# visinf/veto

Hardware: AMD Instinct MI355X
Metric: relation-pairs/sec (PredCls, 36 obj/img) (higher is better)
Workload: dtype fp16 + e4m3 correction terms (fp16 MFMA main product, e4m3 K=128 MFMA cross terms, fp32 accumulate); 1 GPU; BASELINE.json configs[1]: synthetic PredCls, 12 img x 36 obj = 15120 pairs/GPU, d=576, 8 heads, 4 layers, 51 predicates; images_per_gpu=12, objects_per_image=36, pairs_per_gpu=15120, layers=4, heads=8, precision=mixed, parallelism=single GPU

## Files before the change

veto_amd/csrc/attention.hip:

```cpp
#include "common.h"
#include "kernels.h"

#include <cstdio>
#include <cstdlib>
#include <cstring>

namespace veto {

namespace {

constexpr int kWavesPerBlock = 4;

__global__ __launch_bounds__(256) void attention_kernel(AttnArgs a, int dh, int ldh ) {
  extern __shared__ __attribute__((aligned(16))) char smem_raw[];
  const int lane = threadIdx.x & 63, w = threadIdx.x >> 6;
  const long gw = (long)blockIdx.x * kWavesPerBlock + w;
  const int per_wave = 3 * kTokens * ldh + kTokens * 20;
  float* sq = (float*)smem_raw + (size_t)w * per_wave;
  float* sk = sq + kTokens * ldh;
  float* sv = sk + kTokens * ldh;
  float* sp = sv + kTokens * ldh;
  const bool active = gw < (long)a.n_pair * a.heads;
  const int pair = active ? (int)(gw / a.heads) : 0;
  const int head = active ? (int)(gw % a.heads) : 0;
// ... 72 lines not shown
typedef _Float16 att_f16x8 __attribute__((ext_vector_type(8)));
__device__ __forceinline__ f32x16 att_mfma(const u32x4& a, const u32x4& b, const f32x16& c) {
  return __builtin_amdgcn_mfma_f32_32x32x16_f16(__builtin_bit_cast(att_f16x8, a), __builtin_bit_cast(att_f16x8, b), c, 0, 0, 0);
}
typedef short att_s16x4 __attribute__((ext_vector_type(4)));
typedef short att_s16x8 __attribute__((ext_vector_type(8)));

template <int V> struct IntTag { static constexpr int value = V; };
template <int I, int N, class F>
__device__ __forceinline__ void att_static_for(F&& f) {
  if constexpr (I < N) {
    f(IntTag<I>());
    att_static_for<I + 1, N>(f);
  }
}
constexpr int kAttWpb = 2;
#ifdef VETO_ATT_STAMPS
__device__ unsigned long long g_att_stamps[8192 * 10];
#define ATT_T(k) do { __builtin_amdgcn_sched_barrier(0); unsigned long long t_; asm volatile("s_memtime %0\n\ts_waitcnt lgkmcnt(0)" : "=s"(t_)::"memory"); \
                      __builtin_amdgcn_sched_barrier(0); att_dt[k] = t_ - att_t; att_t = t_; } while (0)
#else
#define ATT_T(k)
#endif
template <int DH, bool TAB = false, bool F24 = false>
__global__ __launch_bounds__(64 * kAttWpb, TAB && DH > 72 ? 2 : 3) void attention_mfma_kernel(AttnArgs a) {
  static_assert(!(TAB && F24), "the per-object form reads fp32 tables");
  saturating_conversions_on();
#ifdef VETO_ATT_STAMPS
  unsigned long long att_t, att_dt[10] = {0, 0, 0, 0, 0, 0, 0, 0, 0, 0};
  asm volatile("s_memtime %0\n\ts_waitcnt lgkmcnt(0)" : "=s"(att_t)::"memory");
#endif
  constexpr int KS = (DH + 15) / 16;
  constexpr int RB = DH * 2 + (DH % 32 == 0 ? 16 : 0);
  constexpr int NT = (DH + 31) / 32;
  constexpr int QK_PLANE = kTokens * RB;
  constexpr int V_PLANE = (kTokens + 1) * RB;
  constexpr int O_BYTES = kTokens * DH * 4;
  constexpr int PHASE2 = 2 * V_PLANE + O_BYTES;
  constexpr int kConstBytes = TAB ? (3 * DH * 4 + 32 * 4) : 0;
  constexpr int kImgBytes = ((4 * QK_PLANE > PHASE2 ? 4 * QK_PLANE : PHASE2) + 64 + 15) & ~15;
  constexpr int WAVE_LDS = kImgBytes + kConstBytes;
  constexpr int CH = DH / 8;
  constexpr int PER_MAT = kTokens * CH;
  constexpr int ROUNDS = (3 * PER_MAT + 63) / 64;
  static_assert(DH % 8 == 0 && QK_PLANE % 16 == 0 && V_PLANE % 16 == 0, "layout");
  __shared__ __attribute__((aligned(16))) char smem[kAttWpb * WAVE_LDS];

  const int lane = threadIdx.x & 63, w = __builtin_amdgcn_readfirstlane(threadIdx.x >> 6);
  const long item = (long)blockIdx.x * kAttWpb + w;
  if (item >= (long)a.n_pair * a.heads) return;
  char* base = smem + w * WAVE_LDS;
  char* q_hi = base;
  char* q_lo = base + QK_PLANE;
  char* k_hi = base + 2 * QK_PLANE;
  char* k_lo = base + 3 * QK_PLANE;
  char* v_hi = base;
  char* v_lo = v_hi + V_PLANE;

  constexpr int PC = DH / 4;
  constexpr int PER_MAT4 = kTokens * PC;
  constexpr int ROUNDS4 = (3 * PER_MAT4 + 63) / 64;
  f32x4 ld[TAB ? 1 : ROUNDS][2];
  f32x4 lt[TAB ? ROUNDS4 : 1], lo_[TAB ? ROUNDS4 : 1];
  const int pair = (int)(item / a.heads);
  const int head = (int)(item % a.heads);
  const float* src0 = a.qkv + (size_t)pair * kTokens * (3 * kDim) + head * DH;
  const float* tab_s = nullptr;
  const float* tab_o = nullptr;
  if constexpr (TAB) {
    tab_s = a.sw + (size_t)a.subj[pair] * kPatchTokens * (3 * kDim) + head * DH;
    tab_o = a.ow + (size_t)a.obj[pair] * kPatchTokens * (3 * kDim) + head * DH;
  }
  constexpr int kLateFrom = TAB ? (2 * PER_MAT4 + 63) / 64 : ROUNDS;
  constexpr int kRounds = TAB ? ROUNDS4 : ROUNDS;
  float* const c2_lds = (float*)(base + kImgBytes);
  float* const rs_lds = c2_lds + 3 * DH;
  if constexpr (TAB) {
    constexpr int NC2 = 3 * DH / 4;
#pragma unroll
    for (int idx0 = 0; idx0 < NC2; idx0 += 64) {
      const int idx = idx0 + lane;
      if (idx < NC2) {
        const int mat = idx / PC, c4 = idx % PC;
        *(f32x4*)(c2_lds + idx * 4) = *(const f32x4*)(a.vec + head * DH + mat * kDim + c4 * 4);
      }
    }
    if (lane < kTokens) rs_lds[lane] = a.stats[((size_t)pair * kTokens + lane) * 2 + 1];
  }
  auto load_round = [&](auto r_tag) {
    constexpr int r = decltype(r_tag)::value;
    const int e = lane + 64 * r;
    if constexpr (TAB) {
      const int mat = e / PER_MAT4, rem = e % PER_MAT4, i = rem / PC, c4 = rem % PC;
      const bool need = e < 3 * PER_MAT4;
      lo_[r] = f32x4{0.f, 0.f, 0.f, 0.f};
      if (need && i >= 1 && i <= kPatchTokens) {
        const unsigned off = (unsigned)(((i - 1) * (3 * kDim) + mat * kDim + c4 * 4) * 4);
        lo_[r] = *(const f32x4*)((const char*)tab_o + off);
        lt[r] = *(const f32x4*)((const char*)tab_s + off);
      } else if (need) {
        const unsigned off = (unsigned)((mat * kDim + c4 * 4) * 4) + (i == 0 ? 0u : (unsigned)(i * (3 * kDim) * 4));
        const char* src = i == 0 ? (const char*)(a.vec + 2 * (3 * kDim) + head * DH) : (const char*)src0;
        lt[r] = *(const f32x4*)(src + off);
      } else {
        lt[r] = f32x4{0.f, 0.f, 0.f, 0.f};
      }
    } else {
    const int mat = e / PER_MAT, rem = e % PER_MAT, i = rem / CH, c = rem % CH;
    const bool need = e < 3 * PER_MAT && !(a.cls_only && mat == 0 && i > 0);
    if (F24 && need) {
      const char* src = (const char*)a.qkv + (((size_t)pair * kTokens + i) * (3 * kDim) + mat * kDim + head * DH + c * 8) * 3;
      typedef u32x4 u32x4_a8 __attribute__((aligned(8)));
      const u32x4 d01 = *(const u32x4_a8*)src;
      const u32x2 d2 = *(const u32x2*)(src + 16);
      ld[r][0] = f32x4{__uint_as_float(d01[0]), __uint_as_float(d01[1]), __uint_as_float(d01[2]), __uint_as_float(d01[3])};
      ld[r][1] = f32x4{__uint_as_float(d2[0]), __uint_as_float(d2[1]), 0.f, 0.f};
    } else if (need) {
      const unsigned off = (unsigned)((mat * kDim + c * 8) * 4) + (unsigned)(i * (3 * kDim) * 4);
      ld[r][0] = *(const f32x4*)((const char*)src0 + off);
      ld[r][1] = *(const f32x4*)((const char*)src0 + off + 16u);
    } else {
      ld[r][0] = f32x4{0.f, 0.f, 0.f, 0.f};
      ld[r][1] = f32x4{0.f, 0.f, 0.f, 0.f};
    }
    }
  };
  att_static_for<0, kLateFrom>(load_round);
  ATT_T(0);
  auto convert = [&](auto phase_tag) {
    constexpr int PHASE = decltype(phase_tag)::value;
    if constexpr (TAB) {
      att_static_for<0, ROUNDS4>([&](auto r_tag) {
        constexpr int r = decltype(r_tag)::value;
        if constexpr (!(PHASE == 0 ? r >= kLateFrom : 64 * r + 63 < 2 * PER_MAT4)) {
          const int e = lane + 64 * r;
          const int mat = e / PER_MAT4, rem = e % PER_MAT4, i = rem / PC, c4 = rem % PC;
          if (e < 3 * PER_MAT4) {
            if ((PHASE == 0 ? r < kLateFrom : r >= kLateFrom) && i >= 1 && i <= kPatchTokens)
              lt[r] = rs_lds[i] * (lt[r] + lo_[r]) + *(const f32x4*)(c2_lds + mat * DH + c4 * 4);
            if (PHASE == 0 ? mat < 2 : mat == 2) {
              uint32_t h0, l0, h1, l1;
              att_split2(lt[r][0], lt[r][1], h0, l0);
              att_split2(lt[r][2], lt[r][3], h1, l1);
              char* dst = (PHASE == 0 ? (mat == 0 ? q_hi : k_hi) : v_hi) + i * RB + c4 * 8;
              *(u32x2*)dst = u32x2{h0, h1};
              *(u32x2*)(dst + (PHASE == 0 ? QK_PLANE : V_PLANE)) = u32x2{l0, l1};
            }
          }
        }
      });
    } else {
#pragma unroll
    for (int r = 0; r < ROUNDS; ++r) {
      if (PHASE == 0 ? 64 * r >= 2 * PER_MAT : 64 * r + 63 < 2 * PER_MAT) continue;
      const int e = lane + 64 * r;
      if (e >= 3 * PER_MAT) continue;
      const int mat = e / PER_MAT, rem = e % PER_MAT, i = rem / CH, c = rem % CH;
      if (PHASE == 0 ? mat == 2 : mat < 2) continue;
      f32x4 v0 = ld[r][0], v1 = ld[r][1];
      if constexpr (F24) {
        v0 = unpack_f24x4(__float_as_uint(ld[r][0][0]), __float_as_uint(ld[r][0][1]), __float_as_uint(ld[r][0][2]));
        v1 = unpack_f24x4(__float_as_uint(ld[r][0][3]), __float_as_uint(ld[r][1][0]), __float_as_uint(ld[r][1][1]));
// ... 133 lines not shown
    const int i = e / CH, c = e % CH;
    const f32x4 v0 = *(const f32x4*)(o_lds + i * DH + c * 8);
    const f32x4 v1 = *(const f32x4*)(o_lds + i * DH + c * 8 + 4);
    const size_t row = a.cls_only ? (size_t)pair : (size_t)pair * kTokens + i;
    if (a.o_fmt == FMT_MIXED) {
      store_act8_mixed<true>(a.o + row * (2 * kDim), head * DH + c * 8, v0, v1);
      continue;
    }
    bf16x8 hi, lo;
#pragma unroll
    for (int t = 0; t < 4; ++t) {
      __bf16 hh, ll;
      split_bf16(v0[t], hh, ll);
      hi[t] = hh;
      lo[t] = ll;
      split_bf16(v1[t], hh, ll);
      hi[4 + t] = hh;
      lo[4 + t] = ll;
    }
    __bf16* dst = a.o + row * (2 * kDim) + split_index(head * DH + c * 8);
    *(bf16x8*)dst = hi;
    *(bf16x8*)(dst + 32) = lo;
  }
#ifdef VETO_ATT_STAMPS
  ATT_T(9);
  if (lane == 0) {
    unsigned long long* slot = g_att_stamps + (size_t)(item & 8191) * 10;
    for (int k = 0; k < 10; ++k) slot[k] = att_dt[k];
  }
#endif
}


template <int CTRL>
__device__ __forceinline__ float dpp_rot16(float v) {
  return __int_as_float(__builtin_amdgcn_update_dpp(0, __float_as_int(v), CTRL, 0xF, 0xF, false));
}
__device__ __forceinline__ float row16_sum(float v) {
  v += dpp_rot16<0x128>(v);
  v += dpp_rot16<0x124>(v);
  v += dpp_rot16<0x122>(v);
  v += dpp_rot16<0x121>(v);
  return v;
}

constexpr int kFoldMaxHeads = 12;
// ... 371 lines not shown
      fprintf(stderr, "[cls stamps]");
      for (int k = 1; k <= 12; ++k) fprintf(stderr, " %lld", (long long)(hst[k] - hst[k - 1]));
      fprintf(stderr, "  (request | zero | loads->LN start.. | LN+images | barrier | scores | barrier | softmax | barrier | abar | barrier | staging | stores)\n");
    }
  }
#endif
  return hipGetLastError();
}

bool attention_reads_tables(int heads) {
  if (heads <= 0 || kDim % heads != 0) return false;
  const int dh = kDim / heads;
  return dh == 72 || dh == 96;
}

hipError_t launch_attention(const AttnArgs& a, hipStream_t s) {
  if (kDim % a.heads != 0) return hipErrorInvalidValue;
  const int dh = kDim / a.heads;
  if (dh == 72 || dh == 96) {
    const long items = (long)a.n_pair * a.heads;
    unsigned blocks = (unsigned)((items + kAttWpb - 1) / kAttWpb);
    if (a.sw) {
      if (!a.ow || !a.stats || !a.vec || !a.subj || !a.obj || a.cls_only) return hipErrorInvalidValue;
      if (dh == 72) VETO_LAUNCH((attention_mfma_kernel<72, true>), dim3(blocks), dim3(64 * kAttWpb), 0, s, a);
      else VETO_LAUNCH((attention_mfma_kernel<96, true>), dim3(blocks), dim3(64 * kAttWpb), 0, s, a);
#ifdef VETO_ATT_STAMPS
      {
        static unsigned long long all[8192 * 10];
        unsigned long long host[10] = {0};
        hipDeviceSynchronize();
        hipMemcpyFromSymbol(all, HIP_SYMBOL(g_att_stamps), sizeof(all));
        const long nslots = items < 8192 ? items : 8192;
        for (long i = 0; i < nslots; ++i)
          for (int k = 0; k < 10; ++k) host[k] += all[i * 10 + k];
        const double n = (double)nslots;
        static const char* names[10] = {"issue of the early gathers", "wait for the early gathers", "table arithmetic + Q / K conversion", "issue of the late gathers",
                                        "S^T", "softmax", "wait for the late gathers", "V arithmetic + conversion", "P V + staging", "output conversion + stores"};
        double tot = 0;
        for (int k = 0; k < 10; ++k) tot += host[k] / n;
        fprintf(stderr, "[attention stamps, table form, dh %d, last %.0f items] mean shader-clock cycles per item (s_memtime) and share:\n", dh, n);
        for (int k = 0; k < 10; ++k) fprintf(stderr, "    %-38s %8.1f  %5.1f %%\n", names[k], host[k] / n, 100.0 * host[k] / n / tot);
        fprintf(stderr, "    %-38s %8.1f\n", "sum", tot);
      }
#endif
    } else if (a.qkv_f24) {
      if (dh == 72) VETO_LAUNCH((attention_mfma_kernel<72, false, true>), dim3(blocks), dim3(64 * kAttWpb), 0, s, a);
// ... 25 lines not shown
```

veto_amd/csrc/gemm_split_ps.hip:

```cpp
#include "common.h"
#include "kernels.h"

#include <cstdio>
#include <cstdlib>

namespace veto {

namespace {

constexpr int BM = 256, BN = 192, BK = 32;
constexpr int NCONS = 8, NLOAD = 4;
constexpr int kABytes = BM * 128;
constexpr int kWBytes = BN * 128;
constexpr int kDumpOff = 3 * kABytes + 2 * kWBytes;
constexpr int kBiasOff = kDumpOff + 1024;
constexpr int kBiasSlices = 3;
constexpr int kLdsBytes = kBiasOff + kBiasSlices * BN * 4;
constexpr int kPrefSteps = BN * 4 / 128;
constexpr int CPA = BM / 8 / NLOAD;
constexpr int CPWL = BN / 8 / NLOAD;
#ifndef VETO_GEMM_EPI_T
#define VETO_GEMM_EPI_T 1
#endif
constexpr bool kEpiT = VETO_GEMM_EPI_T;
// ... 21 lines not shown

__device__ __forceinline__ void wg_barrier() {
  asm volatile("" ::: "memory");
  __builtin_amdgcn_s_barrier();
  asm volatile("" ::: "memory");
}

typedef int i32x4 __attribute__((ext_vector_type(4)));
typedef int i32x8 __attribute__((ext_vector_type(8)));
typedef _Float16 f16x8 __attribute__((ext_vector_type(8)));
template <int V> struct IntTag { static constexpr int value = V; };

typedef short s16x4 __attribute__((ext_vector_type(4)));
typedef short s16x8 __attribute__((ext_vector_type(8)));
__device__ __forceinline__ s16x4 lds_tr16(const char* p) {
  return __builtin_amdgcn_ds_read_tr16_b64_v4i16((__attribute__((address_space(3))) s16x4*)p);
}
__device__ __forceinline__ bf16x8 lds_tr_frag(const char* p, int pitch4) {
  const s16x4 a = lds_tr16(p), b = lds_tr16(p + pitch4);
  const s16x8 v = __builtin_shufflevector(a, b, 0, 1, 2, 3, 4, 5, 6, 7);
  return __builtin_bit_cast(bf16x8, v);
}

template <int NTERMS, int EPI_T, bool TN = false>
__global__ __launch_bounds__(64 * (NCONS + NLOAD), 3) void gemm_split_ps_kernel(GemmArgs g) {
  constexpr bool kDrop = EPI_T == EPI_RESID_DROP;
  constexpr bool kMixed = NTERMS == 2;
  if constexpr (kMixed) saturating_conversions_on();
  static_assert(!(kMixed && TN), "the mixed-row format has no transposed (weight-gradient) form");
  constexpr bool kGeluBwd = EPI_T == EPI_GELU_BWD;
  constexpr int EPI = kDrop || kGeluBwd ? (int)EPI_RESID : EPI_T;
  __shared__ __attribute__((aligned(16))) char smem[kLdsBytes];

  const int tid = threadIdx.x;
  const int lane = tid & 63;
  const int w = __builtin_amdgcn_readfirstlane(tid >> 6);
  const int b = blockIdx.x;
  const int ksp = EPI == EPI_ATOMIC && g.k_splits > 1 ? g.k_splits : 1;
  const int out_tiles = g.tiles_m * g.tiles_n;
  const int ntiles = out_tiles * ksp;
  const int K = g.K;
  const int nk = g.kb_tiles > 0 ? g.kb_steps : K / BK / ksp;
  const int per_xcd = gridDim.x >> 3;
  auto tile_of = [&](int it) { return (it * 8 + (b & 7)) * per_xcd + (b >> 3); };
  int my_tiles = 0;
  while (tile_of(my_tiles) < ntiles) ++my_tiles;
  if (my_tiles == 0) return;
// ... 18 lines not shown
      tn_xa[0] = (lane ^ tn_swz(lw)) << 4;
      tn_xa[1] = (lane ^ tn_swz(lw + 8)) << 4;
#pragma unroll
      for (int i = 0; i < CPWL; ++i) {
        const int slot = (lw + NLOAD * i) * 64 + lane, r = slot / 48, cc = slot % 48;
        tn_wr[i] = r;
        tn_wx[i] = (cc ^ tn_swz(r)) << 4;
      }
    }
    auto setupA = [&](int tile) {
      int k0 = (tile / out_tiles) * nk;
      tile %= out_tiles;
      const int tile_m = tile / g.tiles_n;
      if (g.kb_tiles > 0) k0 = ((tile % g.tiles_n) / g.kb_tiles) * nk;
      if constexpr (TN) {
        tnA = (const char*)g.a + (size_t)tile_m * (BM * 4);
        tn_rowA = k0 * BK;
        return;
      }
#pragma unroll
      for (int i = 0; i < CPA; ++i) {
        const int c = lw + NLOAD * i;
        int row = tile_m * BM + c * 8 + rr;
        if (g.lda != 2 * K && row >= g.M) row = g.M - 1;
        srcA[i] = src_of(g.a, g.lda, row, c) + (size_t)k0 * 128;
      }
    };
    auto setupW = [&](int tile) {
      int k0 = (tile / out_tiles) * nk;
      tile %= out_tiles;
      const int tile_n = tile % g.tiles_n;
      if (g.kb_tiles > 0) k0 = (tile_n / g.kb_tiles) * nk;
      if constexpr (TN) {
        tnW = (const char*)g.w + (size_t)tile_n * (BN * 4);
        tn_rowW = k0 * BK;
        return;
      }
#pragma unroll
      for (int i = 0; i < CPWL; ++i) {
        const int c = lw + NLOAD * i;
        srcW[i] = src_of(g.w, 2 * K, tile_n * BN + c * 8 + rr, c) + (size_t)k0 * 128;
      }
    };
    int itA = 0, ktA = 0, bufA = 0, itW = 0, ktW = 0, bufW = 0;
    auto issueA = [&]() {
      if (ktA == 0 && lw == 0 && g.bias && lane < BN / 4) {
        const int tn = (tile_of(itA) % out_tiles) % g.tiles_n;
// ... 222 lines not shown
      if (EPI == EPI_RESID && u < 7) load_res(u + 1, res[(u + 1) & 1]);
      const int row = row0 + m * 16;
#pragma unroll
      for (int j = 0; j < 3; ++j) {
        const int n = h * 3 + j;
        f32x4 t = acc[n][m];
        if (kEpiT) {
#pragma unroll
          for (int e = 0; e < 4; ++e)
            t[e] = __int_as_float(__builtin_amdgcn_ds_bpermute(perm_addr, __float_as_int(acc[n][m][e])));
        }
        if (kGeluBwd) {
          f32x4 v;
#pragma unroll
          for (int e = 0; e < 4; ++e) v[e] = row < g.M ? t[e] * gelu_erf_grad(res[u & 1][j][e]) : 0.f;
          acc[n][m] = v;
        } else if (EPI == EPI_RESID && !kDrop) {
          f32x4 v = t + res[u & 1][j];
          if (g.bias) v += *(const f32x4*)(bias_lds + n * 64);
          acc[n][m] = v;
        } else if (row < g.M) {
          const int col = col0 + n * 16;
          f32x4 v = t;
          if (g.bias) v += *(const f32x4*)(bias_lds + n * 64);
          if (kDrop) {
#pragma unroll
            for (int e = 0; e < 4; ++e)
              v[e] = dropout_keep(g.drop_seed, (unsigned long long)row * g.N + col + e, g.drop_thresh) ? v[e] * g.drop_scale : 0.f;
          }
          if (EPI == EPI_RESID) v += res[u & 1][j];
          if (EPI == EPI_GELU_SPLIT || EPI == EPI_SPLIT) {
            if (EPI == EPI_GELU_SPLIT) {
#pragma unroll
              for (int e = 0; e < 4; ++e) v[e] = gelu_sigmoid(v[e]);
            }
            store_act4<kMixed ? FMT_MIXED : FMT_SPLIT>(g.c_split + (size_t)row * g.ldc, col, v);
          } else if (EPI == EPI_PRE_GELU) {
            *(f32x4*)(g.c + (size_t)row * g.ldc_f32 + col) = v;
#pragma unroll
            for (int e = 0; e < 4; ++e) v[e] = gelu_erf(v[e]);
            store_act4<FMT_SPLIT>(g.c_split + (size_t)row * g.ldc, col, v);
          } else if (EPI == EPI_ATOMIC) {
            float* dstc = g.c + (size_t)row * g.ldc + col;
#pragma unroll
            for (int e = 0; e < 4; ++e) unsafeAtomicAdd(dstc + e, v[e]);
          } else if (EPI == EPI_RESID) {
            acc[n][m] = v;
          } else if (EPI == EPI_F24) {
            *(u32x3*)((char*)g.c + ((size_t)row * g.ldc + col) * 3) = pack_f24x4(v);
          } else {
            *(f32x4*)(g.c + (size_t)row * g.ldc + col) = v;
          }
        }
      }
    }
    if (kGeluBwd) {
      float* cp = g.col_partial + (size_t)(tile_m * 4 + wm) * g.N + col0;
#pragma unroll
      for (int n = 0; n < 6; ++n) {
        f32x4 sum = (acc[n][0] + acc[n][1]) + (acc[n][2] + acc[n][3]);
#pragma unroll
        for (int e = 0; e < 4; ++e) {
          float x = sum[e];
          if (kEpiT) { x += __shfl_xor(x, 4, 64); x += __shfl_xor(x, 8, 64); x += __shfl_xor(x, 16, 64); x += __shfl_xor(x, 32, 64); }
          else { x += __shfl_xor(x, 1, 64); x += __shfl_xor(x, 2, 64); x += __shfl_xor(x, 4, 64); x += __shfl_xor(x, 8, 64); }
          sum[e] = x;
        }
        if (er == 0) *(f32x4*)(cp + n * 16) = sum;
      }
#pragma unroll
      for (int u = 0; u < 8; ++u) {
        const int m = u >> 1, h = u & 1;
// ... 13 lines not shown
        const int row = row0 + m * 16;
        if (row < g.M) {
#pragma unroll
          for (int j = 0; j < 3; ++j) {
            const int n = h * 3 + j;
            *(f32x4*)(g.c + (size_t)row * g.ldc + col0 + n * 16) = acc[n][m];
          }
        }
      }
    }
    STAMP(t3);
    ACC(a_epi, t3, t2);
  }
#ifdef VETO_GEMM_STAMPS
  if (w == 0 && lane == 0) {
    g_stamps[b * 8 + 0] = a_bar; g_stamps[b * 8 + 1] = a_cmp; g_stamps[b * 8 + 2] = a_epi; g_stamps[b * 8 + 3] = t3 - t_begin;
  }
#endif
}

template <int NTERMS>
hipError_t launch_ps_terms(GemmArgs g, int epi, int nblocks, hipStream_t s) {
  dim3 grid(nblocks), block(64 * (NCONS + NLOAD));
  if constexpr (NTERMS == 2) {
    switch (epi) {
      case EPI_F32: VETO_LAUNCH((gemm_split_ps_kernel<2, EPI_F32>), grid, block, 0, s, g); break;
      case EPI_F24: VETO_LAUNCH((gemm_split_ps_kernel<2, EPI_F24>), grid, block, 0, s, g); break;
      case EPI_RESID: VETO_LAUNCH((gemm_split_ps_kernel<2, EPI_RESID>), grid, block, 0, s, g); break;
      case EPI_GELU_SPLIT: VETO_LAUNCH((gemm_split_ps_kernel<2, EPI_GELU_SPLIT>), grid, block, 0, s, g); break;
      default: return hipErrorInvalidValue;
    }
    return hipGetLastError();
  } else
  switch (epi) {
    case EPI_F32: VETO_LAUNCH((gemm_split_ps_kernel<NTERMS, EPI_F32>), grid, block, 0, s, g); break;
    case EPI_F24: VETO_LAUNCH((gemm_split_ps_kernel<NTERMS, EPI_F24>), grid, block, 0, s, g); break;
    case EPI_RESID: VETO_LAUNCH((gemm_split_ps_kernel<NTERMS, EPI_RESID>), grid, block, 0, s, g); break;
    case EPI_GELU_SPLIT: VETO_LAUNCH((gemm_split_ps_kernel<NTERMS, EPI_GELU_SPLIT>), grid, block, 0, s, g); break;
    case EPI_SPLIT: VETO_LAUNCH((gemm_split_ps_kernel<NTERMS, EPI_SPLIT>), grid, block, 0, s, g); break;
    case EPI_PRE_GELU:
      if constexpr (NTERMS == 3) { VETO_LAUNCH((gemm_split_ps_kernel<NTERMS, EPI_PRE_GELU>), grid, block, 0, s, g); break; }
      else return hipErrorInvalidValue;
    case EPI_GELU_BWD:
      if constexpr (NTERMS == 3) {
        if (!g.resid || !g.c_split || !g.col_partial || g.bias) return hipErrorInvalidValue;
        VETO_LAUNCH((gemm_split_ps_kernel<NTERMS, EPI_GELU_BWD>), grid, block, 0, s, g);
// ... 11 lines not shown

}

int gemm_rows_padded(int m) { return (m + BM - 1) / BM * BM; }

hipError_t launch_gemm_split(GemmArgs g, int epi, int precision, hipStream_t s) {
  if (g.N % BN != 0 || g.K % BK != 0 || g.M <= 0) return hipErrorInvalidValue;
  if (g.lda == 0) g.lda = 2 * (long)g.K;
  g.tiles_m = (g.M + BM - 1) / BM;
  g.tiles_n = g.N / BN;
  return launch_gemm_split_ps(g, epi, precision, s);
}

hipError_t launch_gemm_split_ps(GemmArgs g, int epi, int precision, hipStream_t s) {
  int num_cu = device_cu_count();
  if (num_cu < 1) return hipErrorInvalidDevice;
  num_cu = num_cu / 8 * 8;
  if (num_cu < 8) num_cu = 8;
  const int ksp = epi == EPI_ATOMIC && g.k_splits > 1 ? g.k_splits : 1;
  if ((g.K / BK) % ksp != 0) return hipErrorInvalidValue;
  if (g.kb_tiles > 0 && (ksp != 1 || g.tn || g.fmt == FMT_MIXED || g.kb_steps <= 0 || g.tiles_n % g.kb_tiles != 0 ||
                         (g.tiles_n / g.kb_tiles) * g.kb_steps != g.K / BK))
    return hipErrorInvalidValue;
  if (g.tn && (epi != EPI_ATOMIC || !g.zero || g.lda <= 0 || g.ldw <= 0 || g.k_valid <= 0 || g.k_valid > g.K)) return hipErrorInvalidValue;
  const int ntiles = g.tiles_m * g.tiles_n * ksp;
  int nblocks = num_cu;
  if (ntiles < nblocks) nblocks = (ntiles + 7) / 8 * 8;
  if (g.fmt == FMT_MIXED && (g.tn || !g.w_exp || (g.K / BK) % 2 != 0 || ksp != 1)) return hipErrorInvalidValue;
  hipError_t rc = g.fmt == FMT_MIXED ? launch_ps_terms<2>(g, epi, nblocks, s)
                  : precision == 0 ? launch_ps_terms<3>(g, epi, nblocks, s) : launch_ps_terms<1>(g, epi, nblocks, s);
#ifdef VETO_GEMM_STAMPS
  {
    static unsigned long long host[256 * 8];
    hipDeviceSynchronize();
    hipMemcpyFromSymbol(host, HIP_SYMBOL(g_stamps), sizeof(host));
    double sum[8] = {0};
    for (int bb = 0; bb < nblocks && bb < 256; ++bb)
      for (int k = 0; k < 8; ++k) sum[k] += (double)host[bb * 8 + k];
    fprintf(stderr, "[stamps M%d N%d K%d epi%d] consumer: barrier %.0f compute %.0f epilogue %.0f total %.0f | loader: vmwait %.0f "
            "barrier %.0f issue %.0f total %.0f (mean cycles per workgroup; %d tiles x %d k-steps each)\n", g.M, g.N, g.K, epi,
            sum[0] / nblocks, sum[1] / nblocks, sum[2] / nblocks, sum[3] / nblocks, sum[4] / nblocks, sum[5] / nblocks,
            sum[6] / nblocks, sum[7] / nblocks, (ntiles + nblocks - 1) / nblocks, g.K / BK);
  }
#endif
  return rc;
}
// ... 3 lines not shown
```

veto_amd/csrc/kernels.h:

```cpp
#pragma once
#include "common.h"

namespace veto {

enum Epi { EPI_F32 = 0, EPI_RESID = 1, EPI_GELU_SPLIT = 2, EPI_ATOMIC = 3, EPI_RESID_DROP = 4, EPI_F24 = 5, EPI_SPLIT = 6, EPI_PRE_GELU = 7, EPI_GELU_BWD = 8 };

struct GemmArgs {
  const __bf16* a;
  const __bf16* w;
  const float* bias;
  const float* resid;
  float* c;
  __bf16* c_split;
  int M, N, K;
  long lda;
  long ldr;
  long ldc;
  long ldc_f32;
  float* col_partial;
  int k_splits;
  unsigned long long drop_seed;
  unsigned drop_thresh;
  float drop_scale;
  int tiles_m, tiles_n;
  int fmt;
  int kb_tiles, kb_steps;
  const int* w_exp;
  int tn;
  long ldw;
  int k_valid;
  const __bf16* zero;
};

bool env_knob_is(const char* name, const char* value);
int env_knob_int(const char* name, int dflt);
int gemm_rows_padded(int m);
int device_cu_count();
hipError_t launch_gemm_split(GemmArgs g, int epi, int precision, hipStream_t s);
hipError_t launch_gemm_split_ps(GemmArgs g, int epi, int precision, hipStream_t s);

struct FfnArgs {
  const char* a;
  const char* w1;
  const char* w2;
  const float* b1;
  const float* b2;
  const float* resid;
  float* out;
  long ldr, ldo;
  int M;
// ... 78 lines not shown
                               const int32_t* obj, float* qkv, int n_pair, hipStream_t s);
hipError_t launch_qkv0_consts(const float* wq, const float* gamma, const float* beta, const float* pos, const float* cls, float* wp,
                              float* vec, hipStream_t s);
hipError_t launch_dropout_apply(const float* x, float* y, size_t rows, int n_cols, unsigned long long seed, unsigned thresh,
                                float scale, hipStream_t s);

hipError_t launch_count_saturation(const void* base, long stride_bytes, int rows, int K, unsigned long long* counters, hipStream_t s);
hipError_t launch_layernorm(const float* x, long ldx, const float* w, const float* b, __bf16* dst, int rows,
                            hipStream_t s, int fmt = FMT_SPLIT, long ldd = 0, bool x_f24 = false);
hipError_t launch_unpack_f24(const void* src, float* dst, size_t n, hipStream_t s);

struct AttnArgs {
  const float* qkv;
  __bf16* o;
  int n_pair, heads, cls_only;
  int qkv_f24 = 0;
  int o_fmt = FMT_SPLIT;
  const float* sw = nullptr;
  const float* ow = nullptr;
  const float* stats = nullptr;
  const float* vec = nullptr;
  const int32_t* subj = nullptr;
  const int32_t* obj = nullptr;
};
hipError_t launch_attention(const AttnArgs& a, hipStream_t s);
bool attention_reads_tables(int heads);

struct QkvAttnArgs {
  const char* a;
  const char* w;
  const int* w_exp;
  char* o;
  int n_pair, heads;
  int fast;
};
bool qkv_attn_fused_supports(int heads);
size_t qkv_attn_rows_padded(int n_pair);
hipError_t launch_qkv_attn_fused(const QkvAttnArgs& g, hipStream_t s);
int cls_fold_max_heads();
hipError_t launch_cls_fold_attention(const float* x, const float* ln_w, const float* ln_b, const float* u, __bf16* abar, int n_pair, int heads,
                                     hipStream_t s, bool u_f24 = false);
bool cls_fold_reads_f24();

hipError_t launch_head(const float* cls, const float* wt, const float* bias, float* out, int n_pair,
                       int n_out, hipStream_t s, long ld = kDim);

// ... 312 lines not shown
```

veto_amd/csrc/veto_abi.hip:

```cpp
#include <hip/hip_runtime.h>

#include <cstdarg>
#include <cstddef>
#include <cstdio>
#include <cstdlib>
#include <cstring>
#include <atomic>
#include <map>
#include <string>
#include <vector>

#include "../../include/veto_amd.h"
#include "kernels.h"

using namespace veto;

namespace {

thread_local std::string g_err;

int fail(int code, const char* fmt, ...) {
  char buf[512];
  va_list ap;
  va_start(ap, fmt);
// ... 256 lines not shown
  const size_t cpad = (size_t)gemm_rows_padded(chunk);
  w.subj = (int32_t*)take((size_t)n_pair * 4);
  w.obj = (int32_t*)take((size_t)n_pair * 4);
  w.lc = (float*)take((size_t)n_obj * 2 * 2 * kDim * 4);
  w.pa = (__bf16*)take(prow * 2 * 2048 * 2);
  w.patch_tab = (float*)take((size_t)n_obj * 16 * 2 * kDim * 4);
  w.x = (float*)take(mpad * kDim * 4);
  w.a = (__bf16*)take(mpad * 2 * kDim * 2);
  {
    const size_t qkv_bytes = mpad * 3 * kDim * 4, fold_bytes = 2 * (align_up(cpad * (size_t)cls_fold_max_heads() * kDim * 4, 256));
    w.big = take(qkv_bytes > fold_bytes ? qkv_bytes : fold_bytes);
  }
  w.xc = (float*)take(cpad * kDim * 4);
  w.ptab_split = (__bf16*)take(prow * 2 * 2 * kDim * 2);
  w.sw = (float*)take(prow * 3 * kDim * 4);
  w.ow = (float*)take(prow * 3 * kDim * 4);
  w.stats = (float*)take(mpad * 2 * 4);
  w.ac = (__bf16*)take(cpad * 2 * kDim * 2);
  w.hc = (__bf16*)take(cpad * 4 * kDim * 2);
  w.total = off;
  return w;
}

struct DropSite {
  unsigned long long seed = 0;
  unsigned thresh = 0;
  float scale = 1.f;
};

int run_gemm(veto_handle_t h, hipStream_t s, const char* name, const __bf16* a, SplitW w, const float* bias,
             const float* resid, long ldr, float* c, __bf16* c_split, long ldc, int M, int N, int K, int epi,
             long lda = 0, int w_row0 = 0, DropSite drop = DropSite(), const int* w_exp = nullptr, int kb_tiles = 0, int kb_steps = 0) {
  GemmArgs g{};
  g.kb_tiles = kb_tiles; g.kb_steps = kb_steps;
  if (w_exp) { g.fmt = FMT_MIXED; g.w_exp = w_exp; }
  if (drop.thresh) {
    if (epi != EPI_RESID) return fail(VETO_ERR_INVALID, "dropout is fused into the residual epilogue only");
    epi = EPI_RESID_DROP;
    g.drop_seed = drop.seed; g.drop_thresh = drop.thresh; g.drop_scale = drop.scale;
  }
  g.a = a; g.lda = lda;
  g.w = w + (size_t)w_row0 * 2 * K;
  g.bias = bias; g.resid = resid; g.c = c; g.c_split = c_split;
  g.M = M; g.N = N; g.K = K; g.ldr = ldr; g.ldc = ldc;
  if (epi == EPI_PRE_GELU) g.ldc_f32 = N;
  const double kk = kb_tiles > 0 ? 32.0 * kb_steps : (double)K;
  const double flops = 2.0 * M * (double)N * kk;
  const double bytes = 4.0 * ((double)M * K + (double)N * kk) + (double)M * N * (epi == EPI_RESID ? 8.0 : epi == EPI_F24 ? 3.0 : 4.0);
  ProfScope ps(h, s, name, flops, bytes);
  HIP_TRY(launch_gemm_split(g, epi, 0, s));
  return VETO_OK;
}

}

extern "C" {
// ... 239 lines not shown
                      n_obj * 16, 2 * kDim, 2048, EPI_F32);
    if (rc) return rc;
  }
  static const bool tables_off = env_knob_is("VETO_QKV0_TABLES", "0");
  const bool qkv0_tables = L >= 2 && !tables_off;
  static const bool fold_off = env_knob_is("VETO_CLS_FOLD", "0");
  const bool fold_last = !fold_off && H <= cls_fold_max_heads();
  const bool mixed = h->cfg.precision != VETO_PRECISE;
  const bool fast = h->cfg.precision == VETO_FAST;
  const bool mixed_out = mixed && attention_reads_tables(H);
  const bool cls_mixed = mixed;
  static const bool tail_off = env_knob_is("VETO_TAIL_FUSED", "0");
  const bool tail_fused = !tail_off && !sat;
  const bool panel = !sat;
  auto count_sat = [&](int layer, int site, const void* rows, long stride_bytes, int n_rows, int K) -> hipError_t {
    if (!sat) return hipSuccess;
    return launch_count_saturation(rows, stride_bytes, n_rows, K, sat + ((size_t)layer * VETO_SAT_SITES + site) * 4, s);
  };
  static const bool qkv_f24_off = env_knob_is("VETO_QKV_F24", "0");
  static const bool qa_off = env_knob_is("VETO_QKV_ATTN_FUSED", "0");
  const bool qa_fused = mixed && mixed_out && tail_fused && !qa_off && qkv_attn_fused_supports(H);
  static const bool x_f24_on = env_knob_is("VETO_X_F24", "1");
  const bool x_f24 = x_f24_on && !fast && mixed && mixed_out && tail_fused && fold_last && qkv0_tables && qa_fused && L >= 3;
  if (qkv0_tables) {
    const int R = n_obj * 16;
    HIP_TRY(launch_centre_split(ws.patch_tab, ws.ptab_split, R, s));
    int rc = run_gemm(h, s, "gemm_qkv0_tab", ws.ptab_split, h->q0_w, h->q0_vec + 3 * kDim, nullptr, 0, ws.sw, nullptr, 3 * kDim, R, 3 * kDim, kDim,
                      EPI_F32, (long)2 * 2 * kDim, 0);
    if (rc) return rc;
    rc = run_gemm(h, s, "gemm_qkv0_tab", ws.ptab_split + 2 * kDim, h->q0_w, nullptr, nullptr, 0, ws.ow, nullptr, 3 * kDim, R, 3 * kDim, kDim,
                  EPI_F32, (long)2 * 2 * kDim, 0);
    if (rc) return rc;
  }

  for (int c0 = 0; c0 < n_pair; c0 += chunk) {
    const int np = (n_pair - c0 < chunk) ? n_pair - c0 : chunk;
    const int M = np * kTokens;
    float* qkv = (float*)ws.big;
    __bf16* hid = (__bf16*)ws.big;
    {
      AssembleArgs a{};
      a.patch_tab = ws.patch_tab; a.lc = ws.lc; a.cls_token = h->p(T + "cls_token");
      a.pos_embedding = h->p(T + "pos_embedding");
      a.ln_w = h->layers[0].ln1_w; a.ln_b = h->layers[0].ln1_b;
      a.subj = ws.subj + c0; a.obj = ws.obj + c0; a.x = ws.x; a.a = ws.a; a.n_pair = np;
      a.stats = qkv0_tables ? ws.stats : nullptr;
      a.x_f24 = x_f24 ? 1 : 0;
// ... 33 lines not shown
        }
        if (rc) return rc;
        {
          ProfScope ps(h, s, "attention_cls", 4.0 * np * H * kTokens * kDim, (double)M * kDim * 4 + (double)np * H * kDim * 8);
          HIP_TRY(launch_cls_fold_attention(xlast, w.ln1_w, w.ln1_b, u, abar, np, H, s, u24));
        }
        if (dhp > 0) {
          const int hpt = 192 / dhp;
          rc = run_gemm(h, s, "gemm_v_cls", abar, h->fold_v, nullptr, nullptr, 0, nullptr, ws.hc, 2L * npad, np, npad, H * kDim, EPI_SPLIT,
                        0, 0, DropSite(), nullptr, 1, hpt * kDim / 32);
          if (rc) return rc;
          rc = run_gemm(h, s, "gemm_out_cls", ws.hc, h->fold_o, w.out_b, xlast, (long)kTokens * kDim, ws.xc, nullptr, kDim, np, kDim, npad,
                        EPI_RESID);
        } else {
          rc = run_gemm(h, s, "gemm_out_cls", abar, h->fold_n, w.out_b, xlast, (long)kTokens * kDim, ws.xc, nullptr, kDim, np, kDim,
                        H * kDim, EPI_RESID);
        }
        if (rc) return rc;
      } else if (l == 0 && qkv0_tables) {
        if (!attention_reads_tables(H)) {
          ProfScope ps(h, s, "qkv0_combine", 0, (double)np * 17 * 3 * kDim * 4 * 3);
          HIP_TRY(launch_qkv0_combine(ws.sw, ws.ow, ws.stats, h->q0_vec, ws.subj + c0, ws.obj + c0, qkv, np, s));
        }
        for (int t = kTokens - 2; t < kTokens; ++t) {
          if (mixed) HIP_TRY(count_sat(l, VETO_SAT_QKV_IN, ws.a + (size_t)t * 2 * kDim, (long)kTokens * kDim * 4, np, kDim));
          rc = run_gemm(h, s, "gemm_qkv0_lc", ws.a + (size_t)t * 2 * kDim, mixed ? w.qkv_m : w.qkv, nullptr, nullptr, 0,
                        qkv + (size_t)t * 3 * kDim, nullptr, (long)kTokens * 3 * kDim, np, 3 * kDim, kDim, EPI_F32, (long)kTokens * 2 * kDim, 0,
                        DropSite(), mixed ? w.exp_m + 0 : nullptr);
          if (rc) return rc;
        }
      } else if (!last && qa_fused && l > 0) {
        QkvAttnArgs q{};
        q.a = (const char*)ws.a; q.w = (const char*)w.qkv_m; q.w_exp = w.exp_m + 0; q.o = ws.big; q.n_pair = np; q.heads = H; q.fast = fast ? 1 : 0;
        ProfScope ps(h, s, "qkv_attn_fused", 2.0 * M * 3.0 * kDim * kDim + 4.0 * np * kTokens * kTokens * kDim,
                     (double)M * kDim * 8 + 3.0 * kDim * kDim * 4);
        HIP_TRY(launch_qkv_attn_fused(q, s));
        attn_in_big = true;
      } else if (!last) {
        const bool mq = mixed && l > 0;
        qkv_f24 = mq && !qkv_f24_off && attention_reads_tables(H);
        if (mq) HIP_TRY(count_sat(l, VETO_SAT_QKV_IN, ws.a, (long)kDim * 4, M, kDim));
        rc = run_gemm(h, s, "gemm_qkv", ws.a, mq ? w.qkv_m : w.qkv, nullptr, nullptr, 0, qkv, nullptr, 3 * kDim, M, 3 * kDim, kDim,
                      qkv_f24 ? EPI_F24 : EPI_F32, 0, 0, DropSite(), mq ? w.exp_m + 0 : nullptr);
        if (rc) return rc;
      } else {
        rc = run_gemm(h, s, "gemm_kv_last", ws.a, w.qkv, nullptr, nullptr, 0, qkv + kDim, nullptr, 3 * kDim, M, 2 * kDim,
                      kDim, EPI_F32, 0, kDim);
        if (rc) return rc;
        rc = run_gemm(h, s, "gemm_q_cls", ws.a, w.qkv, nullptr, nullptr, 0, qkv, nullptr, (long)kTokens * 3 * kDim, np, kDim,
                      kDim, EPI_F32, (long)kTokens * 2 * kDim, 0);
        if (rc) return rc;
      }
      if (!fold && !attn_in_big) {
        AttnArgs a{};
        a.qkv = qkv; a.n_pair = np; a.heads = H; a.cls_only = last ? 1 : 0;
        a.qkv_f24 = qkv_f24 ? 1 : 0;
        a.o = last ? ws.ac : ws.a;
        a.o_fmt = (!last && mixed_out) ? FMT_MIXED : FMT_SPLIT;
        if (l == 0 && qkv0_tables && attention_reads_tables(H)) {
          a.sw = ws.sw; a.ow = ws.ow; a.stats = ws.stats; a.vec = h->q0_vec; a.subj = ws.subj + c0; a.obj = ws.obj + c0;
        }
        const double nq = last ? 1 : kTokens;
        ProfScope ps(h, s, last ? "attention_cls" : "attention", 4.0 * np * nq * kTokens * kDim,
                     (double)M * 3 * kDim * (qkv_f24 ? 3 : 4) + (double)np * nq * kDim * 4);
        HIP_TRY(launch_attention(a, s));
        if (a.o_fmt == FMT_MIXED) HIP_TRY(count_sat(l, VETO_SAT_ATTN_OUT, ws.a, (long)kDim * 4, M, kDim));
      }
      if (!last) {
        const bool ffn_ln_next = mixed && panel && l + 1 < L - 1;
        if (mixed_out && tail_fused) {
          FfnArgs f{};
          f.a = (const char*)ws.a; f.wo = (const char*)w.out_m; f.bo = w.out_b; f.expo = w.exp_m + 1; f.lnm_w = w.ln2_w; f.lnm_b = w.ln2_b;
          f.w1 = (const char*)w.fc1_m; f.w2 = (const char*)w.fc2_m; f.b1 = w.fc1_b; f.b2 = w.fc2_b; f.exp1 = w.exp_m + 2; f.exp2 = w.exp_m + 3;
          f.resid = ws.x; f.out = ws.x; f.ldr = kDim; f.ldo = kDim; f.M = M; f.ln_out = (char*)ws.a;
          if (attn_in_big) { f.a = ws.big; f.ln_out = ws.big; f.ln1_out = (char*)ws.a; }
          if (ffn_ln_next) { f.ln_w = h->layers[l + 1].ln1_w; f.ln_b = h->layers[l + 1].ln1_b; }
          f.fast = fast ? 1 : 0;
          if (x_f24) {
            f.resid_f24 = 1;
            if (l + 1 < L - 1) f.out_f24 = 1;
            else {
              if (!attn_in_big) return fail(VETO_ERR_INVALID, "internal: 3-byte residual rows without a free buffer for the last tail's fp32 rows");
              f.out = (float*)ws.a;
// ... 1634 lines not shown
```

Before: 1.417 million pairs/s.

## Group consecutive pairs per wave in layer-0 attention and merge qkv0 GEMMs

The layer-0 table-based attention kernel gains a RUN variant in which each wave handles up to eight consecutive pairs for one head. It reloads the subject table only when the subject index changes and stages the constant vectors once per wave, cutting repeated global loads of the shared subject rows. The GEMM kernel gains a row-remapping mode, used to merge the two qkv0 table GEMMs (subject and object halves) into one launch and the two last-token qkv0 GEMMs into one launch. The cost is fewer waves in the attention grid, serial work inside each wave, and a lower occupancy bound of 2 for the RUN variant. The GEMM remap also adds per-row division and modulo in address computation.

```diff
diff --git a/veto_amd/csrc/attention.hip b/veto_amd/csrc/attention.hip
--- a/veto_amd/csrc/attention.hip
+++ b/veto_amd/csrc/attention.hip
@@ -118,9 +118,11 @@
 #else
 #define ATT_T(k)
 #endif
-template <int DH, bool TAB = false, bool F24 = false>
-__global__ __launch_bounds__(64 * kAttWpb, TAB && DH > 72 ? 2 : 3) void attention_mfma_kernel(AttnArgs a) {
+constexpr int kRunCap = 8;
+template <int DH, bool TAB = false, bool F24 = false, bool RUN = false>
+__global__ __launch_bounds__(64 * kAttWpb, RUN || (TAB && DH > 72) ? 2 : 3) void attention_mfma_kernel(AttnArgs a) {
   static_assert(!(TAB && F24), "the per-object form reads fp32 tables");
+  static_assert(TAB || !RUN, "groups of pairs exist in the per-object form only");
   saturating_conversions_on();
 #ifdef VETO_ATT_STAMPS
   unsigned long long att_t, att_dt[10] = {0, 0, 0, 0, 0, 0, 0, 0, 0, 0};
@@ -142,9 +144,9 @@
   static_assert(DH % 8 == 0 && QK_PLANE % 16 == 0 && V_PLANE % 16 == 0, "layout");
   __shared__ __attribute__((aligned(16))) char smem[kAttWpb * WAVE_LDS];
 
-  const int lane = threadIdx.x & 63, w = __builtin_amdgcn_readfirstlane(threadIdx.x >> 6);
+  const int lane_w = threadIdx.x & 63, w = __builtin_amdgcn_readfirstlane(threadIdx.x >> 6);
   const long item = (long)blockIdx.x * kAttWpb + w;
-  if (item >= (long)a.n_pair * a.heads) return;
+  if (item >= (RUN ? (long)((a.n_pair + kRunCap - 1) / kRunCap) : (long)a.n_pair) * a.heads) return;
   char* base = smem + w * WAVE_LDS;
   char* q_hi = base;
   char* q_lo = base + QK_PLANE;
@@ -157,9 +159,31 @@
   constexpr int PER_MAT4 = kTokens * PC;
   constexpr int ROUNDS4 = (3 * PER_MAT4 + 63) / 64;
   f32x4 ld[TAB ? 1 : ROUNDS][2];
-  f32x4 lt[TAB ? ROUNDS4 : 1], lo_[TAB ? ROUNDS4 : 1];
-  const int pair = (int)(item / a.heads);
+  f32x4 lt[TAB ? ROUNDS4 : 1], lo_[TAB && !RUN ? ROUNDS4 : 1];
+  f32x4 ls[RUN ? ROUNDS4 : 1];
+  int pair = RUN ? (int)(item / a.heads) * kRunCap : (int)(item / a.heads);
   const int head = (int)(item % a.heads);
+  const int pair_end = RUN ? (pair + kRunCap < a.n_pair ? pair + kRunCap : a.n_pair) : pair + 1;
+  (void)pair_end;
+  int cur_subj = -1;
+  (void)cur_subj;
+  float* const c2_lds = (float*)(base + kImgBytes);
+  float* const rs_lds = c2_lds + 3 * DH;
+  constexpr int NC2 = 3 * DH / 4;
+  auto stage_c2 = [&]() {
+#pragma unroll
+    for (int idx0 = 0; idx0 < NC2; idx0 += 64) {
+      const int idx = idx0 + lane_w;
+      if (idx < NC2) {
+        const int mat = idx / (DH / 4), c4 = idx % (DH / 4);
+        *(f32x4*)(c2_lds + idx * 4) = *(const f32x4*)(a.vec + head * DH + mat * kDim + c4 * 4);
+      }
+    }
+  };
+  if constexpr (RUN) stage_c2();
+  do {
+  int lane = lane_w;
+  if constexpr (RUN) asm volatile("" : "+v"(lane));
   const float* src0 = a.qkv + (size_t)pair * kTokens * (3 * kDim) + head * DH;
   const float* tab_s = nullptr;
   const float* tab_o = nullptr;
@@ -169,19 +193,23 @@
   }
   constexpr int kLateFrom = TAB ? (2 * PER_MAT4 + 63) / 64 : ROUNDS;
   constexpr int kRounds = TAB ? ROUNDS4 : ROUNDS;
-  float* const c2_lds = (float*)(base + kImgBytes);
-  float* const rs_lds = c2_lds + 3 * DH;
   if constexpr (TAB) {
-    constexpr int NC2 = 3 * DH / 4;
-#pragma unroll
-    for (int idx0 = 0; idx0 < NC2; idx0 += 64) {
-      const int idx = idx0 + lane;
-      if (idx < NC2) {
-        const int mat = idx / PC, c4 = idx % PC;
-        *(f32x4*)(c2_lds + idx * 4) = *(const f32x4*)(a.vec + head * DH + mat * kDim + c4 * 4);
-      }
-    }
+    if constexpr (!RUN) stage_c2();
     if (lane < kTokens) rs_lds[lane] = a.stats[((size_t)pair * kTokens + lane) * 2 + 1];
+  }
+  if constexpr (RUN) {
+    const int sj = a.subj[pair];
+    if (sj != cur_subj) {
+      cur_subj = sj;
+      att_static_for<0, ROUNDS4>([&](auto r_tag) {
+        constexpr int r = decltype(r_tag)::value;
+        const int e = lane + 64 * r;
+        const int mat = e / PER_MAT4, rem = e % PER_MAT4, i = rem / PC, c4 = rem % PC;
+        ls[r] = f32x4{0.f, 0.f, 0.f, 0.f};
+        if (e < 3 * PER_MAT4 && i >= 1 && i <= kPatchTokens)
+          ls[r] = *(const f32x4*)((const char*)tab_s + (unsigned)(((i - 1) * (3 * kDim) + mat * kDim + c4 * 4) * 4));
+      });
+    }
   }
   auto load_round = [&](auto r_tag) {
     constexpr int r = decltype(r_tag)::value;
@@ -189,11 +217,15 @@
     if constexpr (TAB) {
       const int mat = e / PER_MAT4, rem = e % PER_MAT4, i = rem / PC, c4 = rem % PC;
       const bool need = e < 3 * PER_MAT4;
-      lo_[r] = f32x4{0.f, 0.f, 0.f, 0.f};
-      if (need && i >= 1 && i <= kPatchTokens) {
+      if constexpr (!RUN) lo_[r] = f32x4{0.f, 0.f, 0.f, 0.f};
+      if (RUN && need && i >= 1 && i <= kPatchTokens) {
+        lt[r] = *(const f32x4*)((const char*)tab_o + (unsigned)(((i - 1) * (3 * kDim) + mat * kDim + c4 * 4) * 4));
+      } else if (need && i >= 1 && i <= kPatchTokens) {
         const unsigned off = (unsigned)(((i - 1) * (3 * kDim) + mat * kDim + c4 * 4) * 4);
+        if constexpr (!RUN) {
         lo_[r] = *(const f32x4*)((const char*)tab_o + off);
         lt[r] = *(const f32x4*)((const char*)tab_s + off);
+        }
       } else if (need) {
         const unsigned off = (unsigned)((mat * kDim + c4 * 4) * 4) + (i == 0 ? 0u : (unsigned)(i * (3 * kDim) * 4));
         const char* src = i == 0 ? (const char*)(a.vec + 2 * (3 * kDim) + head * DH) : (const char*)src0;
@@ -233,7 +265,11 @@
           const int mat = e / PER_MAT4, rem = e % PER_MAT4, i = rem / PC, c4 = rem % PC;
           if (e < 3 * PER_MAT4) {
             if ((PHASE == 0 ? r < kLateFrom : r >= kLateFrom) && i >= 1 && i <= kPatchTokens)
+            {
+              if constexpr (RUN) lt[r] = rs_lds[i] * (ls[r] + lt[r]) + *(const f32x4*)(c2_lds + mat * DH + c4 * 4);
+              else
               lt[r] = rs_lds[i] * (lt[r] + lo_[r]) + *(const f32x4*)(c2_lds + mat * DH + c4 * 4);
+            }
             if (PHASE == 0 ? mat < 2 : mat == 2) {
               uint32_t h0, l0, h1, l1;
               att_split2(lt[r][0], lt[r][1], h0, l0);
@@ -413,6 +449,8 @@
     *(bf16x8*)dst = hi;
     *(bf16x8*)(dst + 32) = lo;
   }
+  if constexpr (RUN) asm volatile("s_waitcnt lgkmcnt(0)" ::: "memory");
+  } while (RUN && ++pair < pair_end);
 #ifdef VETO_ATT_STAMPS
   ATT_T(9);
   if (lane == 0) {
@@ -830,6 +868,12 @@
     unsigned blocks = (unsigned)((items + kAttWpb - 1) / kAttWpb);
     if (a.sw) {
       if (!a.ow || !a.stats || !a.vec || !a.subj || !a.obj || a.cls_only) return hipErrorInvalidValue;
+      if (a.run_cap) {
+        blocks = (unsigned)(((long)((a.n_pair + kRunCap - 1) / kRunCap) * a.heads + kAttWpb - 1) / kAttWpb);
+        if (dh == 72) VETO_LAUNCH((attention_mfma_kernel<72, true, false, true>), dim3(blocks), dim3(64 * kAttWpb), 0, s, a);
+        else VETO_LAUNCH((attention_mfma_kernel<96, true, false, true>), dim3(blocks), dim3(64 * kAttWpb), 0, s, a);
+        return hipGetLastError();
+      }
       if (dh == 72) VETO_LAUNCH((attention_mfma_kernel<72, true>), dim3(blocks), dim3(64 * kAttWpb), 0, s, a);
       else VETO_LAUNCH((attention_mfma_kernel<96, true>), dim3(blocks), dim3(64 * kAttWpb), 0, s, a);
 #ifdef VETO_ATT_STAMPS
diff --git a/veto_amd/csrc/gemm_split_ps.hip b/veto_amd/csrc/gemm_split_ps.hip
--- a/veto_amd/csrc/gemm_split_ps.hip
+++ b/veto_amd/csrc/gemm_split_ps.hip
@@ -67,7 +67,7 @@
   return __builtin_bit_cast(bf16x8, v);
 }
 
-template <int NTERMS, int EPI_T, bool TN = false>
+template <int NTERMS, int EPI_T, bool TN = false, bool MAP = false>
 __global__ __launch_bounds__(64 * (NCONS + NLOAD), 3) void gemm_split_ps_kernel(GemmArgs g) {
   constexpr bool kDrop = EPI_T == EPI_RESID_DROP;
   constexpr bool kMixed = NTERMS == 2;
@@ -132,7 +132,9 @@
       for (int i = 0; i < CPA; ++i) {
         const int c = lw + NLOAD * i;
         int row = tile_m * BM + c * 8 + rr;
-        if (g.lda != 2 * K && row >= g.M) row = g.M - 1;
+        if ((MAP || g.lda != 2 * K) && row >= g.M) row = g.M - 1;
+        if constexpr (MAP) srcA[i] = src_of(g.a + (size_t)(row / g.map_n) * g.map_a, g.lda, row % g.map_n, c) + (size_t)k0 * 128;
+        else
         srcA[i] = src_of(g.a, g.lda, row, c) + (size_t)k0 * 128;
       }
     };
@@ -401,7 +403,7 @@
         } else if (row < g.M) {
           const int col = col0 + n * 16;
           f32x4 v = t;
-          if (g.bias) v += *(const f32x4*)(bias_lds + n * 64);
+          if (g.bias && (!MAP || row < g.bias_rows)) v += *(const f32x4*)(bias_lds + n * 64);
           if (kDrop) {
 #pragma unroll
             for (int e = 0; e < 4; ++e)
@@ -427,6 +429,8 @@
             acc[n][m] = v;
           } else if (EPI == EPI_F24) {
             *(u32x3*)((char*)g.c + ((size_t)row * g.ldc + col) * 3) = pack_f24x4(v);
+          } else if constexpr (MAP) {
+            *(f32x4*)(g.c + (size_t)(row / g.map_n) * g.map_c + (size_t)(row % g.map_n) * g.ldc + col) = v;
           } else {
             *(f32x4*)(g.c + (size_t)row * g.ldc + col) = v;
           }
@@ -486,6 +490,11 @@
 template <int NTERMS>
 hipError_t launch_ps_terms(GemmArgs g, int epi, int nblocks, hipStream_t s) {
   dim3 grid(nblocks), block(64 * (NCONS + NLOAD));
+  if (g.map_n > 0) {
+    if (epi != EPI_F32) return hipErrorInvalidValue;
+    VETO_LAUNCH((gemm_split_ps_kernel<NTERMS, EPI_F32, false, true>), grid, block, 0, s, g);
+    return hipGetLastError();
+  }
   if constexpr (NTERMS == 2) {
     switch (epi) {
       case EPI_F32: VETO_LAUNCH((gemm_split_ps_kernel<2, EPI_F32>), grid, block, 0, s, g); break;
@@ -543,6 +552,7 @@
   if (g.kb_tiles > 0 && (ksp != 1 || g.tn || g.fmt == FMT_MIXED || g.kb_steps <= 0 || g.tiles_n % g.kb_tiles != 0 ||
                          (g.tiles_n / g.kb_tiles) * g.kb_steps != g.K / BK))
     return hipErrorInvalidValue;
+  if (g.map_n > 0 && (epi != EPI_F32 || g.tn || g.kb_tiles > 0 || g.map_n > g.M)) return hipErrorInvalidValue;
   if (g.tn && (epi != EPI_ATOMIC || !g.zero || g.lda <= 0 || g.ldw <= 0 || g.k_valid <= 0 || g.k_valid > g.K)) return hipErrorInvalidValue;
   const int ntiles = g.tiles_m * g.tiles_n * ksp;
   int nblocks = num_cu;
diff --git a/veto_amd/csrc/kernels.h b/veto_amd/csrc/kernels.h
--- a/veto_amd/csrc/kernels.h
+++ b/veto_amd/csrc/kernels.h
@@ -26,6 +26,9 @@
   int fmt;
   int kb_tiles, kb_steps;
   const int* w_exp;
+  int map_n;
+  long map_a, map_c;
+  int bias_rows;
   int tn;
   long ldw;
   int k_valid;
@@ -150,6 +153,7 @@
   const float* vec = nullptr;
   const int32_t* subj = nullptr;
   const int32_t* obj = nullptr;
+  int run_cap = 0;
 };
 hipError_t launch_attention(const AttnArgs& a, hipStream_t s);
 bool attention_reads_tables(int heads);
diff --git a/veto_amd/csrc/veto_abi.hip b/veto_amd/csrc/veto_abi.hip
--- a/veto_amd/csrc/veto_abi.hip
+++ b/veto_amd/csrc/veto_abi.hip
@@ -302,6 +302,11 @@
   return w;
 }
 
+struct RowMap {
+  int n = 0;
+  long a = 0, c = 0;
+  int bias_rows = 0;
+};
 struct DropSite {
   unsigned long long seed = 0;
   unsigned thresh = 0;
@@ -310,8 +315,10 @@
 
 int run_gemm(veto_handle_t h, hipStream_t s, const char* name, const __bf16* a, SplitW w, const float* bias,
              const float* resid, long ldr, float* c, __bf16* c_split, long ldc, int M, int N, int K, int epi,
-             long lda = 0, int w_row0 = 0, DropSite drop = DropSite(), const int* w_exp = nullptr, int kb_tiles = 0, int kb_steps = 0) {
+             long lda = 0, int w_row0 = 0, DropSite drop = DropSite(), const int* w_exp = nullptr, int kb_tiles = 0, int kb_steps = 0,
+             RowMap map = RowMap()) {
   GemmArgs g{};
+  g.map_n = map.n; g.map_a = map.a; g.map_c = map.c; g.bias_rows = map.bias_rows;
   g.kb_tiles = kb_tiles; g.kb_steps = kb_steps;
   if (w_exp) { g.fmt = FMT_MIXED; g.w_exp = w_exp; }
   if (drop.thresh) {
@@ -597,7 +604,14 @@
   const bool qa_fused = mixed && mixed_out && tail_fused && !qa_off && qkv_attn_fused_supports(H);
   static const bool x_f24_on = env_knob_is("VETO_X_F24", "1");
   const bool x_f24 = x_f24_on && !fast && mixed && mixed_out && tail_fused && fold_last && qkv0_tables && qa_fused && L >= 3;
-  if (qkv0_tables) {
+  static const bool merge_off = env_knob_is("VETO_QKV0_MERGE", "0");
+  if (qkv0_tables && !merge_off) {
+    const int R = n_obj * 16;
+    HIP_TRY(launch_centre_split(ws.patch_tab, ws.ptab_split, R, s));
+    int rc = run_gemm(h, s, "gemm_qkv0_tab", ws.ptab_split, h->q0_w, h->q0_vec + 3 * kDim, nullptr, 0, ws.sw, nullptr, 3 * kDim, 2 * R, 3 * kDim, kDim,
+                      EPI_F32, (long)2 * 2 * kDim, 0, DropSite(), nullptr, 0, 0, RowMap{R, (long)2 * kDim, (long)(ws.ow - ws.sw), R});
+    if (rc) return rc;
+  } else if (qkv0_tables) {
     const int R = n_obj * 16;
     HIP_TRY(launch_centre_split(ws.patch_tab, ws.ptab_split, R, s));
     int rc = run_gemm(h, s, "gemm_qkv0_tab", ws.ptab_split, h->q0_w, h->q0_vec + 3 * kDim, nullptr, 0, ws.sw, nullptr, 3 * kDim, R, 3 * kDim, kDim,
@@ -677,6 +691,15 @@
           ProfScope ps(h, s, "qkv0_combine", 0, (double)np * 17 * 3 * kDim * 4 * 3);
           HIP_TRY(launch_qkv0_combine(ws.sw, ws.ow, ws.stats, h->q0_vec, ws.subj + c0, ws.obj + c0, qkv, np, s));
         }
+        if (!merge_off) {
+          const int t = kTokens - 2;
+          if (mixed)
+            for (int j = 0; j < 2; ++j) HIP_TRY(count_sat(l, VETO_SAT_QKV_IN, ws.a + (size_t)(t + j) * 2 * kDim, (long)kTokens * kDim * 4, np, kDim));
+          rc = run_gemm(h, s, "gemm_qkv0_lc", ws.a + (size_t)t * 2 * kDim, mixed ? w.qkv_m : w.qkv, nullptr, nullptr, 0,
+                        qkv + (size_t)t * 3 * kDim, nullptr, (long)3 * kDim, 2 * np, 3 * kDim, kDim, EPI_F32, (long)2 * kDim, 0,
+                        DropSite(), mixed ? w.exp_m + 0 : nullptr, 0, 0, RowMap{2, (long)kTokens * 2 * kDim, (long)kTokens * 3 * kDim, 0});
+          if (rc) return rc;
+        } else
         for (int t = kTokens - 2; t < kTokens; ++t) {
           if (mixed) HIP_TRY(count_sat(l, VETO_SAT_QKV_IN, ws.a + (size_t)t * 2 * kDim, (long)kTokens * kDim * 4, np, kDim));
           rc = run_gemm(h, s, "gemm_qkv0_lc", ws.a + (size_t)t * 2 * kDim, mixed ? w.qkv_m : w.qkv, nullptr, nullptr, 0,
@@ -714,6 +737,8 @@
         a.o_fmt = (!last && mixed_out) ? FMT_MIXED : FMT_SPLIT;
         if (l == 0 && qkv0_tables && attention_reads_tables(H)) {
           a.sw = ws.sw; a.ow = ws.ow; a.stats = ws.stats; a.vec = h->q0_vec; a.subj = ws.subj + c0; a.obj = ws.obj + c0;
+          static const bool runs_off = env_knob_is("VETO_ATTN_RUNS", "0");
+          a.run_cap = !runs_off && (long)n_pair >= 2L * n_obj ? 1 : 0;
         }
         const double nq = last ? 1 : kTokens;
         ProfScope ps(h, s, last ? "attention_cls" : "attention", 4.0 * np * nq * kTokens * kDim,
```

Result: slower. 1.395 million pairs/s (-1.6%).
